# ishine/zerovox.cpp

Hardware: AMD Instinct MI355X
Metric: audio-seconds/wall-second (xRT) end-to-end phoneme->22.05 kHz wav (higher is better)
Workload: dtype f16*f16->f32 (MFMA) convs, f32 (MFMA) attention/linear, f32 activations

## Files before the change

### zerovox.cpp_amd/csrc/conv.hip

```cpp
#include "kernels.h"
#include "knobs.h"
#include "mfma_common.h"

#include <hip/hip_fp16.h>
#include <algorithm>
#include <cstdlib>
#include <cstring>

namespace zv
{

static constexpr int CK_MAX = 256;
#ifndef ZV_STAGE_U
#define ZV_STAGE_U 4
#endif
#ifndef ZV_STAGE_US
#define ZV_STAGE_US 9
#endif
#ifndef ZV_SINGLE_LW
#define ZV_SINGLE_LW 4
#endif
#ifndef ZV_STAGE_ULW
#define ZV_STAGE_ULW 10
#endif
#ifndef ZV_NT2_OCC
#define ZV_NT2_OCC 3
#endif

int conv_pick_ck(int Cin_p, int ck_max)
{
    if (ck_max <= 0 || ck_max > CK_MAX) ck_max = CK_MAX;
    return Cin_p < ck_max ? Cin_p : ck_max;
}

size_t packed_conv_weight_halfs(int Cin_p, int Cout_p, int K)
{
    return (size_t)((Cout_p + 31) / 32) * K * (Cin_p / 16) * 512;
}

void pack_conv_weight(const uint16_t *w, int K, int IC, int OC, int Cin_p, int Cout_p, int ck, uint16_t *dst)
{
    const int ntiles = (Cout_p + 31) / 32, nicb = Cin_p / 16;
    for (int nt = 0; nt < ntiles; nt++)
        for (int c0 = 0; c0 < Cin_p; c0 += ck)
        {
            const int nkc = ((Cin_p - c0 < ck) ? (Cin_p - c0) : ck) / 16;
            for (int tap = 0; tap < K; tap++)
                for (int kc = 0; kc < nkc; kc++)
                {
                    size_t blk = (size_t)nt * K * nicb + (size_t)K * (c0 / 16) + (size_t)tap * nkc + kc;
                    uint16_t *d = dst + blk * 512;
                    for (int lane = 0; lane < 64; lane++)
                        for (int j = 0; j < 8; j++)
                        {
                            int oc = nt * 32 + (lane & 31);
                            int ic = c0 + kc * 16 + 8 * (lane >> 5) + j;
                            d[lane * 8 + j] = (oc < OC && ic < IC) ? w[((size_t)oc * IC + ic) * K + tap] : (uint16_t)0;
                        }
                }
        }
}

struct StageSrc
{
    const void  *x0, *x1, *x2;
    const float *pa, *pb, *pstat;
    int          ldx, L;
    float        slope, pscale;
};

template <int U, int PRO, int NTH = 256>
__device__ __forceinline__ void stage_tile_p(const StageSrc &J, char *smem, int RS, int c0, int ck, int row_t0, int rows,
                                             int tid)
{
    const int cols = ck >> 2;
    const int total = rows * cols;
    const int L = J.L;
    constexpr int pro = PRO;
    int r = tid / cols, c4 = tid - r * cols;
    const int dr = NTH / cols, dc = NTH - dr * cols;
    const bool hoist = dc == 0;
    float4 hp0 = {0, 0, 0, 0}, hp1 = hp0, hp2 = hp0, hp3 = hp0;
    if (hoist)
    {
        const int c = c0 + c4 * 4;
        if constexpr (pro == PRO_NORM_ACT)
        {
            hp0 = *(const float4 *)(J.pstat + 2 * c);
            hp1 = *(const float4 *)(J.pstat + 2 * c + 4);
            hp2 = *(const float4 *)(J.pa + c);
            hp3 = *(const float4 *)(J.pb + c);
        }
        else if constexpr (pro == PRO_MELNORM)
        {
            hp2 = *(const float4 *)(J.pa + c);
            hp3 = *(const float4 *)(J.pb + c);
        }
    }
    for (int base = tid; base < total; base += NTH * U)
    {
        float4 v[U], v1[U], v2[U];
        half4 hraw[U];
        int lofs[U];
        bool live[U], inr[U];
#pragma unroll
        for (int u = 0; u < U; u++)
        {
            live[u] = base + u * NTH < total;
            const int t = row_t0 + r;
            inr[u] = live[u] && t >= 0 && t < L;
            lofs[u] = r * RS + c4 * 8;
            const size_t off = (size_t)(inr[u] ? t : 0) * J.ldx + c0 + c4 * 4;
            if constexpr (pro == PRO_RAW_F16)
                hraw[u] = *(const half4 *)((const _Float16 *)J.x0 + off);
            else
            {
                v[u] = *(const float4 *)((const float *)J.x0 + off);
                if constexpr (pro == PRO_SUM3_ACT)
                {
                    v1[u] = *(const float4 *)((const float *)J.x1 + off);
                    v2[u] = *(const float4 *)((const float *)J.x2 + off);
                }
            }
            r += dr;
            c4 += dc;
            if (c4 >= cols) { c4 -= cols; r++; }
        }
#pragma unroll
        for (int u = 0; u < U; u++)
        {
            if (!live[u]) continue;
            half4 h = {0, 0, 0, 0};
            if (inr[u])
            {
                if constexpr (pro == PRO_RAW_F16)
                    h = hraw[u];
                else
                {
                    float4 x = v[u];
                    const int c = c0 + ((lofs[u] % RS) >> 1);
                    (void)c;
                    if constexpr (pro == PRO_SUM3_ACT)
                    {
                        const float sc = J.pscale;
                        x.x = ((x.x + v1[u].x) + v2[u].x) * sc;
                        x.y = ((x.y + v1[u].y) + v2[u].y) * sc;
                        x.z = ((x.z + v1[u].z) + v2[u].z) * sc;
                        x.w = ((x.w + v1[u].w) + v2[u].w) * sc;
                    }
                    else if constexpr (pro == PRO_SCALE_ACT)
                    {
                        const float sc = J.pscale;
                        x.x = x.x * sc;
                        x.y = x.y * sc;
                        x.z = x.z * sc;
                        x.w = x.w * sc;
                    }
                    else if constexpr (pro == PRO_NORM_ACT)
                    {
                        float4 st0 = hp0, st1 = hp1, g = hp2, b = hp3;
                        if (!hoist)
                        {
                            st0 = *(const float4 *)(J.pstat + 2 * c);
                            st1 = *(const float4 *)(J.pstat + 2 * c + 4);
                            g = *(const float4 *)(J.pa + c);
                            b = *(const float4 *)(J.pb + c);
                        }
                        x.x = ((x.x - st0.x) * st0.y) * g.x + b.x;
                        x.y = ((x.y - st0.z) * st0.w) * g.y + b.y;
                        x.z = ((x.z - st1.x) * st1.y) * g.z + b.z;
                        x.w = ((x.w - st1.z) * st1.w) * g.w + b.w;
                    }
                    else if constexpr (pro == PRO_MELNORM)
                    {
                        float4 a = hp2, b = hp3;
                        if (!hoist)
// ... 275 lines not shown
#pragma unroll
    for (int mt = 0; mt < MT; mt++) a0[mt] = *(const half8 *)(ap + mt * 32 * RS);

#define ZV_A_ADDR(un) ((un) == 8 ? apn : tb[((un) / NKC) % 4] + ((un) % NKC) * 32)
#define ZV_LOAD_A(dst, un)                                                                   \
    {                                                                                        \
        const char *np_ = ZV_A_ADDR(un);                                                     \
        _Pragma("unroll") for (int mt = 0; mt < MT; mt++) dst[mt] = *(const half8 *)(np_ + mt * 32 * RS); \
    }
    for (int ib = 0; ib < nb; ib++)
    {
        const char *tb[4];
        tb[0] = ap;
#pragma unroll
        for (int x = 1; x < 4; x++) tb[x] = (x < TPB) ? ap + x * dilRS : ap;
        const char *apn = HALF ? ((ib & 1) ? ap + (dilRS - 256) : ap + 256) : ap + TPB * dilRS;
#pragma unroll
        for (int u = 0; u < 4; u++)
#pragma unroll
            for (int nt = 0; nt < NT; nt++) b1[u][nt] = wq[nt * wseg + u * 64];
        __builtin_amdgcn_sched_barrier(0);
        ZV_LOAD_A(a1, 1) mfma_step<MT, NT, SWAP>(acc, a0, b0[0]);
        ZV_LOAD_A(a0, 2) mfma_step<MT, NT, SWAP>(acc, a1, b0[1]);
        ZV_LOAD_A(a1, 3) mfma_step<MT, NT, SWAP>(acc, a0, b0[2]);
        ZV_LOAD_A(a0, 4) mfma_step<MT, NT, SWAP>(acc, a1, b0[3]);
#pragma unroll
        for (int u = 0; u < 4; u++)
#pragma unroll
            for (int nt = 0; nt < NT; nt++) b0[u][nt] = wq[nt * wseg + (4 + u) * 64];
        __builtin_amdgcn_sched_barrier(0);
        ZV_LOAD_A(a1, 5) mfma_step<MT, NT, SWAP>(acc, a0, b1[0]);
        ZV_LOAD_A(a0, 6) mfma_step<MT, NT, SWAP>(acc, a1, b1[1]);
        ZV_LOAD_A(a1, 7) mfma_step<MT, NT, SWAP>(acc, a0, b1[2]);
        ZV_LOAD_A(a0, 8) mfma_step<MT, NT, SWAP>(acc, a1, b1[3]);
        ap = apn;
        wq += 8 * 64;
    }
    if (nsb & 1)
    {
        const char *tb[4] = {ap, ap, ap, ap};
        const char *apn = ap;
        (void)apn;
        ZV_LOAD_A(a1, 1) mfma_step<MT, NT, SWAP>(acc, a0, b0[0]);
        ZV_LOAD_A(a0, 2) mfma_step<MT, NT, SWAP>(acc, a1, b0[1]);
        ZV_LOAD_A(a1, 3) mfma_step<MT, NT, SWAP>(acc, a0, b0[2]);
        mfma_step<MT, NT, SWAP>(acc, a1, b0[3]);
    }
#undef ZV_LOAD_A
#undef ZV_A_ADDR
}


template <int CP, int MT, int NT>
__device__ __forceinline__ void mfma_taps_ring4(floatx16 (&acc)[MT][NT], const char *ap, int dilRS, const half8 *wq, size_t wseg, int K)
{
    constexpr int RS = CP * 2 + 16, NKC = CP / 16;
    static_assert(NKC >= 8, "whole 8-step bodies per tap");
    constexpr bool HALF = NKC == 16;
    const int nb = (K * NKC) >> 3;
    half8 b[4][NT];
#pragma unroll
    for (int u = 0; u < 4; u++)
#pragma unroll
        for (int nt = 0; nt < NT; nt++) b[u][nt] = wq[nt * wseg + u * 64];
    half8 a0[MT], a1[MT];
#pragma unroll
    for (int mt = 0; mt < MT; mt++) a0[mt] = *(const half8 *)(ap + mt * 32 * RS);
#define ZV_R4_LOADA(dst, un)                                                                  \
    {                                                                                         \
        const char *np_ = (un) == 8 ? apn : ap + (un) * 32;                                   \
        _Pragma("unroll") for (int mt = 0; mt < MT; mt++) dst[mt] = *(const half8 *)(np_ + mt * 32 * RS); \
    }
#define ZV_R4_STEP(u, acur, anext)                                                            \
    ZV_R4_LOADA(anext, (u) + 1)                                                               \
    mfma_step<MT, NT, false>(acc, acur, b[(u) & 3]);                                          \
    _Pragma("unroll") for (int nt = 0; nt < NT; nt++) b[(u) & 3][nt] = wq[nt * wseg + ((u) + 4) * 64]; \
    __builtin_amdgcn_sched_barrier(0);
    for (int ib = 0; ib < nb; ib++)
    {
        const char *apn = HALF ? ((ib & 1) ? ap + (dilRS - 256) : ap + 256) : ap + dilRS;
        ZV_R4_STEP(0, a0, a1) ZV_R4_STEP(1, a1, a0) ZV_R4_STEP(2, a0, a1) ZV_R4_STEP(3, a1, a0)
        ZV_R4_STEP(4, a0, a1) ZV_R4_STEP(5, a1, a0) ZV_R4_STEP(6, a0, a1) ZV_R4_STEP(7, a1, a0)
        ap = apn;
        wq += 8 * 64;
    }
#undef ZV_R4_STEP
#undef ZV_R4_LOADA
}

template <int MT>
__device__ __forceinline__ void preload_ring16(half8 (&b)[16], const half8 *wq)
{
#pragma unroll
    for (int u = 0; u < 16; u++) b[u] = wq[u * 64];
}

template <int MT>
__device__ __forceinline__ void mfma_taps_single256(floatx16 (&acc)[MT][1], const char *ap, int dilRS, const half8 *wq, int K,
                                                    half8 (&b)[16])
{
    constexpr int RS = 256 * 2 + 16;
    half8 a[8][MT];
#define ZV_SA(un) (((un) >= 16 ? apn : ap) + ((un) & 15) * 32)
#define ZV_SLOAD(un)                                                                              \
    {                                                                                             \
        const char *np_ = ZV_SA(un);                                                              \
        _Pragma("unroll") for (int mt = 0; mt < MT; mt++) a[(un) & 7][mt] = *(const half8 *)(np_ + mt * 32 * RS); \
    }
#define ZV_SSTEP(u)                                                                               \
    {                                                                                             \
        half8 ac_[MT];                                                                            \
        _Pragma("unroll") for (int mt = 0; mt < MT; mt++) ac_[mt] = a[(u) & 7][mt];               \
        ZV_SLOAD((u) + 6)                                                                         \
        _Pragma("unroll") for (int mt = 0; mt < MT; mt++)                                         \
            acc[mt][0] = __builtin_amdgcn_mfma_f32_32x32x16_f16(ac_[mt], b[u], acc[mt][0], 0, 0, 0); \
        b[u] = wq[(16 + (u)) * 64];                                                               \
        __builtin_amdgcn_sched_barrier(0);                                                        \
    }
    {
        const char *apn = ap;
        ZV_SLOAD(0) ZV_SLOAD(1) ZV_SLOAD(2) ZV_SLOAD(3) ZV_SLOAD(4) ZV_SLOAD(5)
    }
    for (int tap = 0; tap < K; tap++)
    {
        const char *apn = ap + dilRS;
        ZV_SSTEP(0) ZV_SSTEP(1) ZV_SSTEP(2) ZV_SSTEP(3) ZV_SSTEP(4) ZV_SSTEP(5) ZV_SSTEP(6) ZV_SSTEP(7)
        ZV_SSTEP(8) ZV_SSTEP(9) ZV_SSTEP(10) ZV_SSTEP(11) ZV_SSTEP(12) ZV_SSTEP(13) ZV_SSTEP(14) ZV_SSTEP(15)
        ap = apn;
        wq += 16 * 64;
    }
#undef ZV_SSTEP
#undef ZV_SLOAD
#undef ZV_SA
}

__device__ __forceinline__ void l2_warm(const void *base, size_t bytes, int part, int nparts, int tid, int nth)
{
    const size_t lines = (bytes + 127) >> 7;
    const size_t per = (lines + nparts - 1) / nparts, l0 = (size_t)part * per;
    const size_t l1 = l0 + per < lines ? l0 + per : lines;
    unsigned sink = 0;
    for (size_t l = l0 + tid; l < l1; l += nth) sink ^= *(const volatile unsigned *)((const char *)base + (l << 7));
    asm volatile("" ::"v"(sink));
}

template <int MT, int WN, int NT, bool SINGLE = false>
__global__ __launch_bounds__(SINGLE ? 256 + 64 * ZV_SINGLE_LW : 256, (NT == 2 && ZV_NT2_OCC == 3) ? 3 : 2) void conv1d_mfma_kernel(const ConvJobs jobs)
{
    constexpr int WM = 4 / WN;
    constexpr int LW = SINGLE ? ZV_SINGLE_LW : 0;
    constexpr int BM = 32 * MT * WM;
    const ConvJob &J = jobs.j[blockIdx.z];
    int bx = blockIdx.x, by = blockIdx.y, ny = gridDim.y;
    if constexpr (SINGLE)
        if (jobs.xcd_ny)
        {
            const int q = blockIdx.x >> 3, g = q / jobs.xcd_nx;
            by = (blockIdx.x & 7) + 8 * g;
            bx = q - g * jobs.xcd_nx;
            ny = jobs.xcd_ny;
            if (by >= ny) return;
        }

    const int useg = bx / jobs.tps;
    const Seg sg = seg_at(jobs.segs, useg);
    const int L = sg.rows * jobs.rate;
    const int m0 = (bx - useg * jobs.tps) * BM;
    if (m0 >= L) return;
    const size_t row0 = (size_t)sg.row0 * jobs.rate;

    extern __shared__ __attribute__((aligned(16))) char smem[];

    const int tid = threadIdx.x;
    const int lane = tid & 63;
    const int wave = __builtin_amdgcn_readfirstlane(tid >> 6);
    const int wm = wave / WN, wn = wave % WN;

    const int K = J.K, dil = J.dil, Cin_p = J.Cin_p, Cout_p = J.Cout_p;
    const int nicb = Cin_p >> 4;
    const int ntiles = (Cout_p + 31) >> 5;
    const int nt_span = ntiles - jobs.nt_begin;
    const int gt0 = jobs.nt_begin + (int)((long)by * nt_span / ny), gt1 = jobs.nt_begin + (int)((long)(by + 1) * nt_span / ny);
    const int nt0 = gt0 + wn * NT;
    const bool n_ok = nt0 < gt1;
    const int ntl = nt0 + NT <= gt1 ? nt0 : (gt1 - NT > 0 ? gt1 - NT : 0);
    const int rows = BM + (K - 1) * dil;
    const int RS = J.ck * 2 + 16;
    if constexpr (SINGLE)
        if (jobs.xcd_ny && jobs.warm)
            l2_warm((const char *)J.w + (size_t)gt0 * K * nicb * 1024, (size_t)(gt1 - gt0) * K * nicb * 1024, bx, jobs.xcd_nx, tid, 256 + 64 * LW);

    StageSrc S;
    {
        const size_t xo = row0 * J.ldx * (J.pro == PRO_RAW_F16 ? 2 : 4);
        S.x0 = (const char *)J.x0 + xo;
        S.x1 = J.x1 ? (const char *)J.x1 + xo : nullptr;
        S.x2 = J.x2 ? (const char *)J.x2 + xo : nullptr;
        S.pa = J.pa ? J.pa + (size_t)useg * J.pab_seg : nullptr;
        S.pb = J.pb ? J.pb + (size_t)useg * J.pab_seg : nullptr;
        S.pstat = J.pstat ? J.pstat + (size_t)useg * J.pstat_seg : nullptr;
        S.ldx = J.ldx;
        S.L = L;
        S.slope = J.slope;
        S.pscale = J.pscale;
    }

    floatx16 acc[MT][NT];
#pragma unroll
    for (int i = 0; i < MT; i++)
#pragma unroll
        for (int n = 0; n < NT; n++)
#pragma unroll
            for (int r = 0; r < 16; r++) acc[i][n][r] = 0.f;

    const char *abase = smem + (wm * 32 * MT + (lane & 31)) * RS + (lane >> 5) * 16;

    half8 bring[SINGLE ? 16 : 1];
    const bool single256 = SINGLE && NT == 1 && J.ck == 256 && Cin_p >= 256 && n_ok;
#ifdef ZV_STAMPS
    const int stamp_wg = bx + jobs.tps * jobs.segs.nseg * by;
    int stamp_k = 1;
#endif
    ZV_STAMP(0)
    if constexpr (LW > 0)
        if (wave >= 4)
        {
            constexpr int NL = 64 * (LW > 0 ? LW : 1), UL = ZV_STAGE_ULW;
            const int ltid = tid - 256;
            const bool split = J.pro != PRO_SUM3_ACT && rows * (J.ck >> 2) <= NL * UL && !(ZV_DBGBITS(J.dbg) & 1);
            StageRegs<UL> Ra, Rb;
            const int nck = J.ck;
            auto ckof = [&](int c) { return (Cin_p - c < nck) ? (Cin_p - c) : nck; };
#define ZV_LOAD_(P) stage_load_p<UL, P, NL>(S, cn_, ckn_, m0 - J.pad, rows, ltid, R_)
#define ZV_STORE_(P) stage_store_p<UL, P, NL>(S, dst_, RS, cn_, ckn_, m0 - J.pad, rows, ltid, R_)
#define ZV_LD_TILE(REGS, c)                                        \
    if ((c) < Cin_p)                                               \
    {                                                              \
        StageRegs<UL> &R_ = REGS;                                  \
        const int cn_ = (c), ckn_ = ckof(c);                       \
        ZV_STAGE_SPLIT_SWITCH(J.pro, ZV_LOAD_)                     \
    }
#define ZV_ST_TILE(REGS, c, buf)                                   \
    if ((c) < Cin_p)                                               \
    {                                                              \
        const StageRegs<UL> &R_ = REGS;                            \
        const int cn_ = (c), ckn_ = ckof(c);                       \
        char *dst_ = smem + (buf) * jobs.tile_bytes;               \
        ZV_STAGE_SPLIT_SWITCH(J.pro, ZV_STORE_)                    \
    }
#define ZV_RAW_BARRIER()                                           \
    asm volatile("s_waitcnt lgkmcnt(0)" ::: "memory");             \
    __builtin_amdgcn_s_barrier();                                  \
    asm volatile("" ::: "memory");
            if (split)
            {
                ZV_LD_TILE(Ra, 0)
                ZV_LD_TILE(Rb, nck)
                ZV_ST_TILE(Ra, 0, 0)
#ifdef ZV_STAMPS_LOADER
                const int stamp_wg = bx + jobs.tps * jobs.segs.nseg * by;
                int lk = 1;
                ZV_STAMP(0)
#define ZV_LSTAMP() if (lk < 11) { asm volatile("s_waitcnt lgkmcnt(0)" ::: "memory"); ZV_STAMP(lk) lk++; }
#else
#define ZV_LSTAMP()
#endif
                for (int c0 = 0; c0 < Cin_p; c0 += 2 * nck)
                {
                    ZV_LD_TILE(Ra, c0 + 2 * nck)
                    ZV_LSTAMP()
                    ZV_RAW_BARRIER()
                    ZV_LSTAMP()
                    ZV_ST_TILE(Rb, c0 + nck, 1)
                    ZV_LSTAMP()
                    if (c0 + nck >= Cin_p) break;
                    ZV_LD_TILE(Rb, c0 + 3 * nck)
                    ZV_LSTAMP()
                    ZV_RAW_BARRIER()
                    ZV_LSTAMP()
                    ZV_ST_TILE(Ra, c0 + 2 * nck, 0)
                    ZV_LSTAMP()
                }
#ifdef ZV_STAMPS_LOADER
                ZV_STAMP(11)
#endif
#undef ZV_LSTAMP
            }
            else
            {
                int par = 0;
                for (int c0 = 0; c0 < Cin_p; c0 += J.ck)
                {
                    const int ck = ckof(c0);
                    if (!(ZV_DBGBITS(J.dbg) & 1))
                        stage_tile<ZV_STAGE_ULW, NL>(J.pro, S, smem + par * jobs.tile_bytes, RS, c0, ck, m0 - J.pad, rows, ltid);
                    __syncthreads();
                    par ^= 1;
                }
            }
#undef ZV_RAW_BARRIER
#undef ZV_ST_TILE
#undef ZV_LD_TILE
#undef ZV_LOAD_
#undef ZV_STORE_
            return;
        }
    if constexpr (SINGLE)
        if (single256) preload_ring16<MT>(bring, (const half8 *)J.w + (size_t)ntl * K * nicb * 64 + lane);
    int par = 0;
    for (int c0 = 0; c0 < Cin_p; c0 += J.ck)
    {
        const int ck = (Cin_p - c0 < J.ck) ? (Cin_p - c0) : J.ck;
        if (LW == 0 && c0) __syncthreads();
        if (LW == 0 && !(ZV_DBGBITS(J.dbg) & 1))
        {
            if (J.pro == PRO_RAW_F16 && (ck & 7) == 0 && !SINGLE)
                stage_raw16<(BM >= 64 ? 9 : 5), 256>(S, smem, RS, c0, ck, m0 - J.pad, rows, tid);
            else
                stage_tile<(SINGLE ? ZV_STAGE_US : (MT * NT >= 4 ? 8 : ZV_STAGE_U))>(J.pro, S, smem, RS, c0, ck, m0 - J.pad, rows, tid);
        }
        if constexpr (LW > 0)
        {
            asm volatile("s_waitcnt lgkmcnt(0)" ::: "memory");
            __builtin_amdgcn_s_barrier();
            asm volatile("" ::: "memory");
        }
        else
            __syncthreads();
#ifdef ZV_STAMPS
        if (stamp_k < 10) { ZV_STAMP(stamp_k) stamp_k++; }
#endif
        if (n_ok && !(ZV_DBGBITS(J.dbg) & 2))
        {
            const char *ab_ = abase + (LW > 0 ? par * jobs.tile_bytes : 0);
            const half8 *wp = (const half8 *)J.w + ((size_t)ntl * K * nicb + (size_t)K * (c0 >> 4)) * 64 + lane;
            const size_t wseg = (size_t)K * nicb * 64;
            if constexpr (SINGLE && NT == 1)
            {
                if (ck == 256 && single256)
                    mfma_taps_single256<MT>(acc, ab_, dil * RS, wp, K, bring);
                else
                    mfma_chunk<MT, NT>(acc, ab_, RS, dil, wp, wseg, K, ck >> 4);
            }
            else if constexpr (NT == 2)
            {
                if (ck == 256 && J.ck == 256)
                    mfma_taps_ring4<256, MT, NT>(acc, ab_, dil * RS, wp, wseg, K);
                else
                    mfma_chunk<MT, NT>(acc, ab_, RS, dil, wp, wseg, K, ck >> 4);
            }
            else if (ck == 256 && J.ck == 256)
                mfma_taps<256, MT, NT, false>(acc, ab_, dil * RS, wp, wseg, K);
            else if (ck == 128 && J.ck == 128)
                mfma_taps<128, MT, NT, false>(acc, ab_, dil * RS, wp, wseg, K);
            else if (ck == 64 && J.ck == 64)
                mfma_taps<64, MT, NT, false>(acc, ab_, dil * RS, wp, wseg, K);
            else
                mfma_chunk<MT, NT>(acc, ab_, RS, dil, wp, wseg, K, ck >> 4);
        }
#ifdef ZV_STAMPS
        if (stamp_k < 11) { ZV_STAMP(stamp_k) stamp_k++; }
#endif
        par ^= 1;
    }

    if (!n_ok || (ZV_DBGBITS(J.dbg) & 4)) return;
    const float escale = J.escale;
    const int tbase = m0 + wm * 32 * MT + 4 * (lane >> 5);
    const bool has_res = J.res != nullptr;
    const float *res = has_res ? J.res + row0 * J.ldres : nullptr;
    const size_t out0 = row0 * J.ldo;
#pragma unroll
    for (int n = 0; n < NT; n++)
    {
        const int nt = ntl + n;
        if (nt < nt0) continue;
        const int oc = nt * 32 + (lane & 31);
        if (oc >= Cout_p) continue;
        const float bias = J.bias ? J.bias[oc] : 0.f;
        float resv[MT][16];
        if (has_res)
        {
#pragma unroll
            for (int mt = 0; mt < MT; mt++)
#pragma unroll
                for (int r = 0; r < 16; r++)
                {
                    const int t = tbase + mt * 32 + (r & 3) + 8 * (r >> 2);
                    resv[mt][r] = res[(size_t)(t < L ? t : L - 1) * J.ldres + oc];
                }
        }
#pragma unroll
        for (int mt = 0; mt < MT; mt++)
        {
            float outv[16];
#pragma unroll
            for (int r = 0; r < 16; r++)
            {
                const int t = tbase + mt * 32 + (r & 3) + 8 * (r >> 2);
                float v = acc[mt][n][r] + bias;
                if (has_res) v = v + resv[mt][r];
                v = v * escale;
                if (J.eact) v = lrelu(v, J.oslope);
                outv[r] = v;
                if (t < L)
                {
                    if constexpr (SINGLE)
                    {
                        if (J.out_f16) ((_Float16 *)J.out)[out0 + (size_t)t * J.ldo + oc] = (_Float16)v;
                        else ((float *)J.out)[out0 + (size_t)t * J.ldo + oc] = v;
                    }
                    else
                    if (J.out_f16)
                        __builtin_nontemporal_store((_Float16)v, (_Float16 *)J.out + out0 + (size_t)t * J.ldo + oc);
                    else
                        __builtin_nontemporal_store(v, (float *)J.out + out0 + (size_t)t * J.ldo + oc);
                }
            }
            if (J.stat_part && oc < J.stat_C)
            {
                const int blk = (m0 >> 5) + wm * MT + mt;
                if (blk * 32 < L)
                    tile_stats_store(outv, tbase + mt * 32, L, J.stat_part + (((size_t)useg * J.stat_nblk + blk) * J.stat_C + oc) * 2);
            }
        }
    }
#ifdef ZV_STAMPS
    asm volatile("s_waitcnt vmcnt(0)" ::: "memory");
    ZV_STAMP(11)
#endif
}

template <int MT, int WN, int NT, bool SINGLE = false>
static hipError_t launch_cfg(hipStream_t s, ConvJobs &jobs, int njobs, int Lmax, int Cout_p, int halo, int ck, int dmax_)
{
    constexpr int WM = 4 / WN;
    constexpr int BM = 32 * MT * WM;
    const int ntiles = (Cout_p + 31) / 32 - jobs.nt_begin;
    jobs.tps = (Lmax + BM - 1) / BM;
    dim3 grid(jobs.tps * jobs.segs.nseg, (ntiles + WN * NT - 1) / (WN * NT), njobs);
#ifdef ZV_STAMPS
    jobs.stamp = knob(ZV_STAMP_CONV) && knob(ZV_STAMP_CONV) == (int)grid.y && njobs == 1 &&
                         (knob(ZV_STAMP_CIN) ? jobs.j[0].Cin_p == knob(ZV_STAMP_CIN) : jobs.j[0].Cin_p >= 1024)
                     ? stamp_buffer()
                     : nullptr;
#endif
    constexpr int LW = SINGLE ? ZV_SINGLE_LW : 0;
    jobs.xcd_ny = 0;
    jobs.warm = knob(ZV_CONV_WARM) != 0;
    if (SINGLE && knob(ZV_CONV_XCD) != 0)
    {
        jobs.xcd_ny = grid.y;
        jobs.xcd_nx = grid.x;
        grid = dim3(8 * grid.x * ((grid.y + 7) / 8), 1, njobs);
    }
    jobs.tile_bytes = round_up((BM + halo + dmax_) * (ck * 2 + 16), 16);
    const size_t lds = (size_t)jobs.tile_bytes * (LW > 0 ? 2 : 1);
    if (lds > 160 * 1024) return hipErrorInvalidValue;
    return launch_lds(conv1d_mfma_kernel<MT, WN, NT, SINGLE>, grid, dim3(256 + 64 * LW), lds, s, jobs);
}

hipError_t launch_conv_gemm(hipStream_t s, const ConvJob &job, const Segs &segs, int rate);

template <int NKC>
__global__ __launch_bounds__(256, NKC == 8 ? 2 : 3) void conv_stream_kernel(const ConvJobs jobs, const int strip)
{
    constexpr int K = 3, CIN = 16 * NKC, RS = CIN * 2 + 16, NF = K * NKC, TROWS = 64 + K - 1;
    constexpr int C4 = CIN / 4, NP = (TROWS * C4 + 255) / 256, TILE_B = TROWS * RS;
    const ConvJob &J = jobs.j[0];
    const int useg = blockIdx.x / jobs.tps;
    const Seg sg = seg_at(jobs.segs, useg);
    const int L = sg.rows * jobs.rate;
    const int s0 = (blockIdx.x - useg * jobs.tps) * strip * 64;
    if (s0 >= L) return;
    const size_t row0 = (size_t)sg.row0 * jobs.rate;
    extern __shared__ __attribute__((aligned(16))) char smem[];
    const int tid = threadIdx.x, lane = tid & 63;
    const int wave = __builtin_amdgcn_readfirstlane(tid >> 6);
    const int ntiles = (J.Cout_p + 31) >> 5;
    const int nt_w = blockIdx.y * 4 + wave;
    const bool n_ok = nt_w < ntiles;
    const int nt = n_ok ? nt_w : ntiles - 1;
    half8 wf[NF];
    {
        const half8 *wp = (const half8 *)J.w + (size_t)nt * NF * 64 + lane;
#pragma unroll
        for (int i = 0; i < NF; i++) wf[i] = wp[i * 64];
    }
    const int oc = nt * 32 + (lane & 31);
    const float bias = J.bias ? J.bias[oc] : 0.f;
    const float *xs = (const float *)J.x0 + row0 * J.ldx;
    float *outp = (float *)J.out + row0 * J.ldo;
    const float sc = J.pro == PRO_ACT ? 1.0f : J.pscale, sl = J.slope;
    const int pad = J.pad;

    float4 v[NP];
    auto load_tile = [&](int m0) {
#pragma unroll
        for (int p = 0; p < NP; p++)
        {
            const int idx = tid + p * 256 < TROWS * C4 ? tid + p * 256 : TROWS * C4 - 1;
            const int r = idx / C4, c4 = idx % C4;
            const int t = m0 - pad + r;
            v[p] = *(const float4 *)(xs + (size_t)(t < 0 ? 0 : (t < L ? t : L - 1)) * J.ldx + c4 * 4);
        }
    };
    auto write_tile = [&](int buf, int m0) {
#pragma unroll
        for (int p = 0; p < NP; p++)
        {
            const int idx = tid + p * 256;
            if (idx >= TROWS * C4) continue;
            const int r = idx / C4, c4 = idx % C4;
            const int t = m0 - pad + r;
            float4 x = v[p];
            x.x = x.x * sc;
            x.y = x.y * sc;
            x.z = x.z * sc;
            x.w = x.w * sc;
            half4 h;
            h[0] = (_Float16)lrelu(x.x, sl);
            h[1] = (_Float16)lrelu(x.y, sl);
            h[2] = (_Float16)lrelu(x.z, sl);
            h[3] = (_Float16)lrelu(x.w, sl);
            uint2 pk = *(uint2 *)&h;
            const bool in = t >= 0 && t < L;
            pk.x = in ? pk.x : 0u;
            pk.y = in ? pk.y : 0u;
            *(uint2 *)(smem + buf * TILE_B + r * RS + c4 * 8) = pk;
        }
    };

    int m0 = s0;
    load_tile(m0);
    write_tile(0, m0);
    __syncthreads();
    const char *abase = smem + (lane & 31) * RS + (lane >> 5) * 16;
    for (int i = 0; i < strip && m0 < L; i++, m0 += 64)
    {
        const bool more = i + 1 < strip && m0 + 64 < L;
        if (more) load_tile(m0 + 64);
        __builtin_amdgcn_sched_barrier(0);
        floatx16 acc[2];
        const floatx16 z = {0.f, 0.f, 0.f, 0.f, 0.f, 0.f, 0.f, 0.f, 0.f, 0.f, 0.f, 0.f, 0.f, 0.f, 0.f, 0.f};
        const char *ab = abase + (i & 1) * TILE_B;
#pragma unroll
        for (int tap = 0; tap < K; tap++)
#pragma unroll
            for (int kc = 0; kc < NKC; kc++)
            {
                const half8 a0 = *(const half8 *)(ab + tap * RS + kc * 32);
                const half8 a1 = *(const half8 *)(ab + (32 + tap) * RS + kc * 32);
                const bool first = tap == 0 && kc == 0;
                acc[0] = __builtin_amdgcn_mfma_f32_32x32x16_f16(a0, wf[tap * NKC + kc], first ? z : acc[0], 0, 0, 0);
                acc[1] = __builtin_amdgcn_mfma_f32_32x32x16_f16(a1, wf[tap * NKC + kc], first ? z : acc[1], 0, 0, 0);
            }
        if (n_ok)
        {
            const int tbase = m0 + 4 * (lane >> 5);
#pragma unroll
            for (int mt = 0; mt < 2; mt++)
#pragma unroll
                for (int r = 0; r < 16; r++)
                {
                    const int t = tbase + mt * 32 + (r & 3) + 8 * (r >> 2);
                    const float vv = (acc[mt][r] + bias) * J.escale;
                    if (t < L) __builtin_nontemporal_store(vv, outp + (size_t)t * J.ldo + oc);
                }
        }
        if (more) write_tile((i + 1) & 1, m0 + 64);
        __syncthreads();
    }
}

static bool conv_stream_ok(const ConvJob &j, int njobs, int nt_begin)
{
    return njobs == 1 && nt_begin == 0 && (j.pro == PRO_ACT || j.pro == PRO_SCALE_ACT) && j.K == 3 && j.dil == 1 && j.pad == 1 &&
           (j.Cin_p == 64 || j.Cin_p == 128) && j.ck == j.Cin_p && (j.ldx & 3) == 0 && !j.res && !j.stat_part && !j.eact && !j.out_f16 &&
           !j.x1 && !j.x2;
}

static hipError_t launch_conv_stream(hipStream_t s, const ConvJob &job, int n_cu, const Segs &segs, int rate)
{
    ConvJobs js;
    js.j[0] = job;
    js.j[0].dbg = diag_bits();
    for (int i = 1; i < CONV_MAX_JOBS; i++) js.j[i] = js.j[0];
    js.segs = segs;
    js.rate = rate;
    js.nt_begin = 0;
    js.order = 0;
    const int Lmax = segs.max_rows * rate;
    const int ntiles = (job.Cout_p + 31) / 32, gy = (ntiles + 3) / 4;
    const int occ = job.Cin_p == 128 ? 2 : 3;
    int strip = 8;
    while (strip > 2 && (long)((Lmax + 64 * strip - 1) / (64 * strip)) * segs.nseg * gy < 12L * occ * n_cu) strip >>= 1;
    js.tps = (Lmax + 64 * strip - 1) / (64 * strip);
    const dim3 grid(js.tps * segs.nseg, gy, 1);
    const size_t lds = (size_t)2 * 66 * (job.Cin_p * 2 + 16);
    if (job.Cin_p == 128)
        hipLaunchKernelGGL(conv_stream_kernel<8>, grid, dim3(256), lds, s, js, strip);
    else
        hipLaunchKernelGGL(conv_stream_kernel<4>, grid, dim3(256), lds, s, js, strip);
    return hipGetLastError();
}

static hipError_t launch_conv_from(hipStream_t s, const ConvJob *jobs, int njobs, int n_cu, const Segs &segs, int rate, int nt_begin);

hipError_t launch_conv(hipStream_t s, const ConvJob *jobs, int njobs, int n_cu, const Segs &segs, int rate)
{
    if (njobs < 1 || njobs > CONV_MAX_JOBS || segs.nseg < 1 || segs.max_rows < 1) return hipErrorInvalidValue;
    {
        const int g_env = knob(ZV_CONV_GEMM);
        const long rows = (long)segs.max_rows * rate * segs.nseg;
        ConvJob rest[CONV_MAX_JOBS];
        int nrest = 0, ngemm = 0;
        for (int i = 0; i < njobs; i++)
        {
            const ConvJob &j = jobs[i];
            const bool ok = g_env != 0 && (g_env == 2 || rows >= 16384) && j.w8 && j.pro == PRO_RAW_F16 && j.Cin_p >= 128 &&
                            conv_gemm_groups(j.Cout_p) >= 1 && !j.out_f16 && (j.ldx & 7) == 0;
            if (!ok)
            {
                rest[nrest++] = j;
                continue;
            }
            ngemm++;
            hipError_t e = launch_conv_gemm(s, j, segs, rate);
            if (e != hipSuccess) return e;
            const int done = conv_gemm_tiles(j.Cout_p);
            if (done * 32 < j.Cout_p)
            {
                e = launch_conv_from(s, &j, 1, n_cu, segs, rate, done);
                if (e != hipSuccess) return e;
            }
        }
        if (ngemm) return nrest ? launch_conv_from(s, rest, nrest, n_cu, segs, rate, 0) : hipSuccess;
    }
    return launch_conv_from(s, jobs, njobs, n_cu, segs, rate, 0);
}

static hipError_t launch_conv_from(hipStream_t s, const ConvJob *jobs, int njobs, int n_cu, const Segs &segs, int rate, int nt_begin)
{
    const int dbg = diag_bits();
    ConvJobs js;
    js.segs = segs;
    js.rate = rate;
    js.tps = 0;
    js.nt_begin = nt_begin;
    js.order = 0;
    const int Lmax = segs.max_rows * rate;
    int halo = 0, ck = 0, dmax = 1;
    for (int i = 0; i < njobs; i++)
    {
        js.j[i] = jobs[i];
        dmax = jobs[i].dil > dmax ? jobs[i].dil : dmax;
        js.j[i].dbg = dbg;
        if (jobs[i].Cout_p != jobs[0].Cout_p) return hipErrorInvalidValue;
        const int h = (jobs[i].K - 1) * jobs[i].dil;
        if (h > halo) halo = h;
        ck = jobs[i].ck > ck ? jobs[i].ck : ck;
        if (jobs[i].stat_part && jobs[i].stat_nblk * 32 < Lmax) return hipErrorInvalidValue;
    }
    for (int i = njobs; i < CONV_MAX_JOBS; i++) js.j[i] = js.j[0];
    const int Cout_p = jobs[0].Cout_p;
    const int ntiles = (Cout_p + 31) / 32 - nt_begin;
    if (ntiles < 1) return hipErrorInvalidValue;
    const int WN = ntiles >= 3 ? 4 : (ntiles >= 2 ? 2 : 1);
    auto wgs = [&](int MT, int NT) {
        const int BM = 32 * MT * (4 / WN);
        return (long)((Lmax + BM - 1) / BM) * segs.nseg * ((ntiles + WN * NT - 1) / (WN * NT)) * njobs;
    };
    int MT = 4;
    while (MT > 1 && wgs(MT, 1) < 2L * n_cu) MT >>= 1;
    while (MT > 1 && (size_t)(32 * MT * (4 / WN) + halo + dmax) * (ck * 2 + 16) > 80 * 1024) MT >>= 1;
    {
        const double ai = 2.0 * jobs[0].K * jobs[0].Cin_p * Cout_p / (4.0 * (jobs[0].Cin_p + Cout_p));
        const int st_env = knob(ZV_CONV_STREAM);
        if (st_env && conv_stream_ok(jobs[0], njobs, nt_begin) && (st_env == 2 || (ai < 200.0 && wgs(1, 1) >= 16L * n_cu)))
            return launch_conv_stream(s, jobs[0], n_cu, segs, rate);
        if (ai < 200.0 && wgs(1, 1) >= 16L * n_cu) MT = std::min(MT, 2);
    }
    if (MT < knob(ZV_CONV_MT)) MT = knob(ZV_CONV_MT);
    const int nt_env = knob(ZV_CONV_NT);
    int NT = (WN == 4 && ntiles >= 8 && MT >= 2 && wgs(MT, 2) >= 4L * n_cu && jobs[0].K * jobs[0].Cin_p >= 2048) ? 2 : 1;
    if (nt_env == 1 || (nt_env == 2 && WN == 4 && ntiles >= 2 && MT >= 2)) NT = nt_env;
    if (NT == 2 && MT == 4) MT = 2;
    {
        if (knob(ZV_CONV_SINGLE) != 0 && MT == 1 && NT == 1 && ck == 256 && wgs(1, 1) <= 2L * n_cu &&
            (jobs[0].Cin_p > 256 || knob(ZV_CONV_SINGLE) == 2))
        {
            if (WN == 4) return launch_cfg<1, 4, 1, true>(s, js, njobs, Lmax, Cout_p, halo, ck, dmax);
            if (WN == 2) return launch_cfg<1, 2, 1, true>(s, js, njobs, Lmax, Cout_p, halo, ck, dmax);
        }
    }
#define ZV_CASE(mt, wn, nt) \
    if (MT == mt && WN == wn && NT == nt) return launch_cfg<mt, wn, nt>(s, js, njobs, Lmax, Cout_p, halo, ck, dmax);
    ZV_CASE(4, 4, 1) ZV_CASE(2, 4, 1) ZV_CASE(1, 4, 1) ZV_CASE(2, 4, 2)
    ZV_CASE(4, 2, 1) ZV_CASE(2, 2, 1) ZV_CASE(1, 2, 1)
    ZV_CASE(4, 1, 1) ZV_CASE(2, 1, 1) ZV_CASE(1, 1, 1)
#undef ZV_CASE
    return hipErrorInvalidValue;
}



typedef float f32x4 __attribute__((ext_vector_type(4)));
__device__ __forceinline__ float4 nt_load4(const float *p)
{
    const f32x4 v = __builtin_nontemporal_load((const f32x4 *)p);
    return make_float4(v[0], v[1], v[2], v[3]);
}

__global__ __launch_bounds__(256) void out_conv_tanh_kernel(const OutConvArgs a)
{
    extern __shared__ __attribute__((aligned(16))) char smem[];
    const int Cp = round_up(a.C, 16);
    const int RS = Cp * 2 + 16;
    const int K = a.K, pad = (K - 1) / 2;
    const int rows = 256 + K - 1;
    const int tps = (a.segs.max_rows * a.rate + 255) >> 8;
    const int useg = blockIdx.x / tps;
    const Seg sg = seg_at(a.segs, useg);
    const int L = sg.rows * a.rate;
    const int m0 = (blockIdx.x - useg * tps) * 256;
    if (m0 >= L) return;
    const size_t row0 = (size_t)sg.row0 * a.rate;
    const float *x0 = a.x0 + row0 * a.ldx, *x1 = a.x1 ? a.x1 + row0 * a.ldx : nullptr, *x2 = a.x2 ? a.x2 + row0 * a.ldx : nullptr;
    const int tid = threadIdx.x;
    _Float16 *wl = (_Float16 *)(smem + rows * RS);
    for (int i = tid; i < K * Cp; i += 256) wl[i] = ((const _Float16 *)a.w)[i];

    const int cols = Cp >> 2;
    for (int idx = tid; idx < rows * cols; idx += 256)
    {
        const int r = idx / cols, c4 = idx - r * cols;
        const int t = m0 - pad + r;
        half4 h = {0, 0, 0, 0};
        if (t >= 0 && t < L)
        {
            const size_t off = (size_t)t * a.ldx + c4 * 4;
            float4 v = nt_load4(x0 + off);
            if (x1)
            {
                const float4 b = nt_load4(x1 + off);
                const float4 d = nt_load4(x2 + off);
                v.x = ((v.x + b.x) + d.x) * a.pscale;
                v.y = ((v.y + b.y) + d.y) * a.pscale;
                v.z = ((v.z + b.z) + d.z) * a.pscale;
                v.w = ((v.w + b.w) + d.w) * a.pscale;
            }
            else
            {
                v.x = v.x * a.pscale;
                v.y = v.y * a.pscale;
                v.z = v.z * a.pscale;
                v.w = v.w * a.pscale;
            }
            h[0] = (_Float16)lrelu(v.x, a.slope);
            h[1] = (_Float16)lrelu(v.y, a.slope);
            h[2] = (_Float16)lrelu(v.z, a.slope);
            h[3] = (_Float16)lrelu(v.w, a.slope);
        }
        *(half4 *)(smem + r * RS + c4 * 8) = h;
    }
    __syncthreads();
    const int t = m0 + tid;
    if (t >= L) return;
    float acc = 0.f;
    for (int tap = 0; tap < K; tap++)
    {
        const char *row = smem + (tid + tap) * RS;
        for (int c = 0; c < Cp; c += 8)
        {
            const half8 x = *(const half8 *)(row + c * 2);
            const half8 w = *(const half8 *)(wl + tap * Cp + c);
#pragma unroll
            for (int j = 0; j < 8; j++) acc = fmaf((float)x[j], (float)w[j], acc);
        }
    }
    const int skip = a.runs && t >= (sg.aux + 1) * a.rate ? a.segs.tab[useg].pad * a.rate : 0;
    a.out[row0 + t + skip] = tanhf(acc + a.bias);
}

hipError_t launch_out_conv(hipStream_t s, const OutConvArgs &a)
{
    const int Cp = round_up(a.C, 16);
    const size_t lds = (size_t)(256 + a.K - 1) * (Cp * 2 + 16) + (size_t)a.K * Cp * 2;
    if (lds > 64 * 1024 || a.segs.nseg < 1) return hipErrorInvalidValue;
    const int tps = (a.segs.max_rows * a.rate + 255) / 256;
    hipLaunchKernelGGL(out_conv_tanh_kernel, dim3(tps * a.segs.nseg), dim3(256), lds, s, a);
    return hipGetLastError();
}

}
```

### zerovox.cpp_amd/csrc/kernels.h

```cpp
#pragma once

#include <hip/hip_runtime.h>
#include <stdint.h>

#ifdef ZV_DIAG
#define ZV_DBGBITS(x) (x)
#else
#define ZV_DBGBITS(x) 0
#endif

namespace zv
{

__host__ __device__ static inline int round_up(int x, int a) { return (x + a - 1) / a * a; }

struct Seg
{
    int32_t row0, rows;
    int32_t aux;
    int32_t pad;
};
struct Segs
{
    const Seg *tab;
    int        nseg;
    int        max_rows;
    Seg        one;
};
__host__ __device__ static inline Seg seg_at(const Segs &s, int u)
{
    Seg g = s.tab ? s.tab[u] : s.one;
#if defined(__HIP_DEVICE_COMPILE__)
    g.row0 = __builtin_amdgcn_readfirstlane(g.row0);
    g.rows = __builtin_amdgcn_readfirstlane(g.rows);
    g.aux = __builtin_amdgcn_readfirstlane(g.aux);
#endif
    return g;
}
static inline Segs segs_single(int rows, int aux = 0)
{
    Segs s;
    s.tab = nullptr;
    s.nseg = 1;
    s.max_rows = rows;
    s.one.row0 = 0;
    s.one.rows = rows;
    s.one.aux = aux;
    s.one.pad = 0;
    return s;
}


enum ConvPrologue : int
{
    PRO_RAW_F16 = 0,
    PRO_ACT = 1,
    PRO_NORM_ACT = 2,
    PRO_MELNORM = 3,
    PRO_SUM3_ACT = 4,
    PRO_SCALE_ACT = 5
};

struct ConvJob
{
    const void  *x0, *x1, *x2;
    int          ldx;
    int          pro;
    float        slope, pscale;
    const float *pa, *pb;
    const float *pstat;
    int          L, Cin_p, Cout_p, K, dil, pad;
    int          ck;
    const void  *w;
    const void  *w8;
    const float *bias;
    const float *res;
    int          ldres;
    float        escale;
    int          eact;
    float        oslope;
    int          out_f16;
    void        *out;
    int          ldo;
    int          dbg;
    int          pstat_seg, pab_seg;
    double      *stat_part;
    int          stat_nblk, stat_C;
};

constexpr int CONV_MAX_JOBS = 4;
struct ConvJobs
{
    ConvJob j[CONV_MAX_JOBS];
    Segs    segs;
    int     rate;
    int     tps;
    int     nt_begin;
    int     order;
    int     tile_bytes;
    int     xcd_ny, xcd_nx;
    int     warm;
#ifdef ZV_STAMPS
    unsigned long long *stamp;
#endif
};

size_t packed_conv_weight_halfs(int Cin_p, int Cout_p, int K);
int    conv_pick_ck(int Cin_p, int ck_max = 0);
void   pack_conv_weight(const uint16_t *w, int K, int IC, int OC, int Cin_p, int Cout_p, int ck, uint16_t *dst);
int    conv_gemm_groups(int Cout_p);
int    conv_gemm_tiles(int Cout_p);
int    conv_gemm_units(int Cin_p, int K);
size_t conv_gemm_weight_halfs(int Cin_p, int Cout_p, int K);
void   pack_conv_weight_gemm(const uint16_t *w, int K, int IC, int OC, int Cin_p, int Cout_p, uint16_t *dst);
hipError_t launch_conv(hipStream_t s, const ConvJob *jobs, int njobs, int n_cu, const Segs &segs, int rate);

struct PairJob
{
    const float *y;
    float       *out;
    const void  *w1, *w2;
    const void  *w1r, *w2r;
    const float *b1, *b2;
    int          L, Cp, K, dil;
    float        slope;
    int          dbg;
    const float *sum_in;
    float       *sum_out;
};
constexpr int PAIR_MAX_JOBS = 3;
struct PairJobs
{
    PairJob j[PAIR_MAX_JOBS];
    Segs    segs;
    int     rate;
    int     njobs, kmax;
    int     deal_c;
#ifdef ZV_STAMPS
    unsigned long long *stamp;
#endif
    float  *merge_out;
    int     ring_off;
};
bool       pair_supported(int Cp, int K);
size_t     pair_weight_halfs(int Cp, int K);
void       pack_pair_weight(const uint16_t *w, int K, int C, int Cp, uint16_t *dst);
size_t     pair_weight16_halfs(int Cp, int K);
void       pack_pair_weight16(const uint16_t *w, int K, int C, int Cp, uint16_t *dst, bool conv2_layout);
size_t     pair_ring_weight_halfs(int Cp, int K);
void       pack_pair_weight_ring(const uint16_t *w, int K, int C, int Cp, uint16_t *dst, bool conv2_layout);
hipError_t launch_pair(hipStream_t s, const PairJob *jobs, int njobs, int n_cu, const Segs &segs, int rate, float *merge_out = nullptr);

constexpr int TRIPLE_MAX_DIL = 3;
struct TripleJob
{
    const float *y;
    float       *out;
    const void  *w1[TRIPLE_MAX_DIL], *w2[TRIPLE_MAX_DIL];
    const void  *w1x[TRIPLE_MAX_DIL], *w2x[TRIPLE_MAX_DIL];
    const float *b1[TRIPLE_MAX_DIL], *b2[TRIPLE_MAX_DIL];
    int          dil[TRIPLE_MAX_DIL];
    int          n_dil;
    int          L, Cp, K;
    float        slope;
    int          dbg;
};
struct TripleJobs
{
    TripleJob j[PAIR_MAX_JOBS];
    Segs      segs;
    int       rate;
    int       deal_c;
    int       interleave;
    int       db_mask;
    int       ring_off;
#ifdef ZV_STAMPS
    unsigned long long *stamp;
#endif
};
bool       triple_supported(int Cp, int K, const int *dil, int n_dil);
bool       block64_supported(int Cp, int K, const int *dil, int n_dil);
hipError_t launch_block64(hipStream_t s, const TripleJob *jobs, int njobs, const Segs &segs, int rate);
hipError_t launch_triple(hipStream_t s, const TripleJob *jobs, int njobs, int n_cu, const Segs &segs, int rate);

struct OutConvArgs
{
    const float *x0, *x1, *x2;
    int          ldx, L, C, K;
    float        pscale, slope;
    const uint16_t *w;
    float        bias;
    float       *out;
    Segs         segs;
    int          rate;
    int          runs;
};
hipError_t launch_out_conv(hipStream_t s, const OutConvArgs &a);

hipError_t launch_stats_partial(hipStream_t s, const float *x, int ldx, int C, double *part, int nblk, const Segs &segs, int rate);
hipError_t launch_stats_finalize(hipStream_t s, const double *part, int nblk, int C, float eps, float *stat, int stat_seg,
                                 int c_off, const Segs &segs, int rate, int dec_runs = 0);
hipError_t launch_norm_apply(hipStream_t s, const float *x, int ldx, int C, const float *stat, int stat_seg, const float *g,
                             const float *b, float *y, int ldy, double *part, int nblk, const Segs &segs);

hipError_t launch_act_f16(hipStream_t s, const float *x0, const float *x1, const float *x2, float pscale, float slope, void *out, size_t n);
hipError_t launch_norm_act_f16(hipStream_t s, const float *x, int ldx, int C, const double *part, int nblk, int Cpart, float eps,
                               float *stat, int stat_seg, const float *ga, const float *be, int gb_seg, float slope, void *y,
                               int ldy, const Segs &segs, void *yraw = nullptr, int dec_runs = 0);

hipError_t launch_linear(hipStream_t s, const float *x, int ldx, int in, const float *W, const float *b, int out, float *y,
                         int ldy, const float *extra, const Segs &segs);

hipError_t launch_embed(hipStream_t s, const int32_t *ids, const int32_t *puncts, const float *wemb, int emb,
                        const float *pemb, int pdim, const float *posenc, float *x, int ld, const Segs &segs);
hipError_t launch_attention(hipStream_t s, const float *q, const float *k, const float *v, int ld, int H, int dk,
                            float inv_temp, float *o, int ldo, const Segs &segs);
constexpr int CTL_STRIDE = 8;
constexpr int CTL_DURATION = 0;
constexpr int CTL_PITCH = 1;
constexpr int CTL_ENERGY = 3;
constexpr int CTL_TARGET = 5;
constexpr int PCTL_STRIDE = 4;
constexpr int PCTL_FRAMES = 0;
constexpr int PCTL_DURATION = 1;
constexpr int PCTL_PITCH = 2;
constexpr int PCTL_ENERGY = 3;

hipError_t launch_add_layernorm(hipStream_t s, const float *x, int ldx, const float *res, int ldr, int C, int Cp,
                                const float *w, const float *b, float eps, float *y, int ldy, const Segs &segs);
bool       layernorm_tail_ok(int C);
hipError_t launch_layernorm_tail(hipStream_t s, const float *x, int ldx, const float *res, int ldr, int C, int Cp, const float *w,
                                 const float *b, float eps, float *y, int ldy, const Segs &segs, const float *post, int post_seg,
                                 const float *dot_w, const float *dot_b, float *pred, const float *emb, int nbins, int embC, float *feat,
                                 int ldf, int32_t *bucket, const float *ctl = nullptr, int ctl_field = 0,
                                 const float *pctl = nullptr);
hipError_t launch_add_rowvec(hipStream_t s, float *x, int ld, int C, const float *v, int v_seg, const Segs &segs);
hipError_t launch_rowdot(hipStream_t s, const float *x, int ld, int C, const float *w, const float *b, float *y, const Segs &segs);
hipError_t launch_bucket_embed_add(hipStream_t s, const float *pred, int nbins, const float *emb, int C, float *x, int ld,
                                   int32_t *bucket, const Segs &segs, const float *ctl = nullptr, int ctl_field = 0,
                                   const float *pctl = nullptr);
hipError_t launch_length_regulator(hipStream_t s, const float *feat, int ld, const float *logdur, int C, float *hidden,
                                   int ldh, int32_t *cum, int32_t *n_frames, const Segs &tokens, const Segs &frames,
                                   const float *ctl = nullptr, const float *pctl = nullptr);

constexpr int FIT_MAX_TOKENS = 3584;
hipError_t launch_fit_durations(hipStream_t s, const float *logdur, const float *ctl, const float *pctl, const Segs &tokens,
                                const Segs &frames);

hipError_t launch_live_frames(hipStream_t s, const int32_t *n_frames, Seg *live, const Segs &frames);
hipError_t launch_zero_tail(hipStream_t s, float *x, int C, const Segs &frames, const Segs &live, int rate);

constexpr int VOC_RUN_MARGIN = 16;
hipError_t launch_voc_runs(hipStream_t s, const float *mel, int M, float *mel_c, int32_t *eq, Seg *runs, const Segs &frames, int H);
// ... 7 lines not shown
```

Before: 33340.

## Spread XCD-pinned conv blocks across chiplets for multi-segment batches and reroute large batches

```diff
diff --git a/zerovox.cpp_amd/csrc/conv.hip b/zerovox.cpp_amd/csrc/conv.hip
--- a/zerovox.cpp_amd/csrc/conv.hip
+++ b/zerovox.cpp_amd/csrc/conv.hip
@@ -1,3 +1,4 @@
+#include "conv_xcd.h"
 #include "kernels.h"
 #include "knobs.h"
 #include "mfma_common.h"
@@ -22,6 +23,9 @@
 #endif
 #ifndef ZV_STAGE_ULW
 #define ZV_STAGE_ULW 10
+#endif
+#ifndef ZV_CONV_BATCH_ROUTE
+#define ZV_CONV_BATCH_ROUTE 1
 #endif
 #ifndef ZV_NT2_OCC
 #define ZV_NT2_OCC 3
@@ -603,14 +607,17 @@
     constexpr int BM = 32 * MT * WM;
     const ConvJob &J = jobs.j[blockIdx.z];
     int bx = blockIdx.x, by = blockIdx.y, ny = gridDim.y;
+    int warm_part = 0, warm_parts = 1;
     if constexpr (SINGLE)
         if (jobs.xcd_ny)
         {
-            const int q = blockIdx.x >> 3, g = q / jobs.xcd_nx;
-            by = (blockIdx.x & 7) + 8 * g;
-            bx = q - g * jobs.xcd_nx;
+            ConvXcdSlot slot;
+            if (!conv_xcd_slot(blockIdx.x, jobs.xcd_nx, jobs.xcd_ny, jobs.xcd_spread, slot)) return;
+            bx = slot.bx;
+            by = slot.by;
             ny = jobs.xcd_ny;
-            if (by >= ny) return;
+            warm_part = slot.part;
+            warm_parts = slot.nparts;
         }
 
     const int useg = bx / jobs.tps;
@@ -639,7 +646,7 @@
     const int RS = J.ck * 2 + 16;
     if constexpr (SINGLE)
         if (jobs.xcd_ny && jobs.warm)
-            l2_warm((const char *)J.w + (size_t)gt0 * K * nicb * 1024, (size_t)(gt1 - gt0) * K * nicb * 1024, bx, jobs.xcd_nx, tid, 256 + 64 * LW);
+            l2_warm((const char *)J.w + (size_t)gt0 * K * nicb * 1024, (size_t)(gt1 - gt0) * K * nicb * 1024, warm_part, warm_parts, tid, 256 + 64 * LW);
 
     StageSrc S;
     {
@@ -897,13 +904,14 @@
                      : nullptr;
 #endif
     constexpr int LW = SINGLE ? ZV_SINGLE_LW : 0;
-    jobs.xcd_ny = 0;
+    jobs.xcd_ny = jobs.xcd_spread = 0;
     jobs.warm = knob(ZV_CONV_WARM) != 0;
     if (SINGLE && knob(ZV_CONV_XCD) != 0)
     {
         jobs.xcd_ny = grid.y;
         jobs.xcd_nx = grid.x;
-        grid = dim3(8 * grid.x * ((grid.y + 7) / 8), 1, njobs);
+        jobs.xcd_spread = jobs.segs.nseg > 1;
+        grid = dim3(conv_xcd_grid(jobs.xcd_nx, jobs.xcd_ny, jobs.xcd_spread), 1, njobs);
     }
     jobs.tile_bytes = round_up((BM + halo + dmax_) * (ck * 2 + 16), 16);
     const size_t lds = (size_t)jobs.tile_bytes * (LW > 0 ? 2 : 1);
@@ -1138,7 +1146,8 @@
     if (nt_env == 1 || (nt_env == 2 && WN == 4 && ntiles >= 2 && MT >= 2)) NT = nt_env;
     if (NT == 2 && MT == 4) MT = 2;
     {
-        if (knob(ZV_CONV_SINGLE) != 0 && MT == 1 && NT == 1 && ck == 256 && wgs(1, 1) <= 2L * n_cu &&
+        const bool batch_rounds = ZV_CONV_BATCH_ROUTE && segs.nseg > 1 && wgs(1, 1) > n_cu;
+        if (knob(ZV_CONV_SINGLE) != 0 && MT == 1 && NT == 1 && ck == 256 && wgs(1, 1) <= 2L * n_cu && !batch_rounds &&
             (jobs[0].Cin_p > 256 || knob(ZV_CONV_SINGLE) == 2))
         {
             if (WN == 4) return launch_cfg<1, 4, 1, true>(s, js, njobs, Lmax, Cout_p, halo, ck, dmax);
diff --git a/zerovox.cpp_amd/csrc/conv_xcd.h b/zerovox.cpp_amd/csrc/conv_xcd.h
--- /dev/null
+++ b/zerovox.cpp_amd/csrc/conv_xcd.h
@@ -0,0 +1,47 @@
+#pragma once
+
+#if defined(__HIPCC__)
+#define ZV_CX_FN __host__ __device__ static inline
+#else
+#define ZV_CX_FN static inline
+#endif
+
+namespace zv
+{
+
+
+ZV_CX_FN int conv_xcd_spread(int ny) { return ny <= 1 ? 8 : (ny == 2 ? 4 : (ny <= 4 ? 2 : 1)); }
+
+ZV_CX_FN int conv_xcd_grid(int nx, int ny, int spread)
+{
+    if (!spread || ny >= 8) return 8 * nx * ((ny + 7) / 8);
+    const int p = conv_xcd_spread(ny);
+    return 8 * ((nx + p - 1) / p);
+}
+
+struct ConvXcdSlot
+{
+    int bx, by, part, nparts;
+};
+
+ZV_CX_FN bool conv_xcd_slot(int b, int nx, int ny, int spread, ConvXcdSlot &s)
+{
+    const int x = b & 7, q = b >> 3;
+    if (!spread || ny >= 8)
+    {
+        const int g = q / nx;
+        s.by = x + 8 * g;
+        s.bx = q - g * nx;
+        s.part = s.bx;
+        s.nparts = nx;
+        return s.by < ny;
+    }
+    const int p = conv_xcd_spread(ny), g = x / p, r = x - g * p;
+    s.by = g;
+    s.bx = q * p + r;
+    s.part = q;
+    s.nparts = (nx - r + p - 1) / p;
+    return g < ny && s.bx < nx;
+}
+
+}
diff --git a/zerovox.cpp_amd/csrc/kernels.h b/zerovox.cpp_amd/csrc/kernels.h
--- a/zerovox.cpp_amd/csrc/kernels.h
+++ b/zerovox.cpp_amd/csrc/kernels.h
@@ -99,6 +99,7 @@
     int     order;
     int     tile_bytes;
     int     xcd_ny, xcd_nx;
+    int     xcd_spread;
     int     warm;
 #ifdef ZV_STAMPS
     unsigned long long *stamp;
```

Measured after the change: 34080 (median of 6 runs). 1.02x the previous value.
